# sm00thix/cvmatrix

Hardware: AMD Instinct MI355X
Metric: folds/sec (training_XTX_XTY, center+scale) at N=1e5,K=512 (higher is better)
Workload: dtype f64

## Files before the change

cvmatrix_amd/_lib.py:

```python

from __future__ import annotations

import ctypes as C
import os

import torch

_HERE = os.path.dirname(os.path.abspath(__file__))
LIB_PATH = os.environ.get("CVM_LIB_PATH") or os.path.join(_HERE, "libcvmhip.so")

CVM_OK, CVM_EINVAL, CVM_EWORKSPACE, CVM_ELAUNCH = 0, 1, 2, 3
CVM_F32, CVM_F64 = 0, 1
RET_XTX, RET_XTY = 0x01, 0x02
CENTER_X, CENTER_Y, SCALE_X, SCALE_Y = 0x04, 0x08, 0x10, 0x20
IDX_HOST = 0x40

EXPORTS = (
    "cvm_version", "cvm_source_hash", "cvm_last_error", "cvm_gstats_len", "cvm_fit_workspace_bytes",
    "cvm_gram_fit", "cvm_fold_workspace_bytes", "cvm_fold_update", "cvm_fold_update_ex", "cvm_plan_fold", "cvm_debug_force_splits", "cvm_debug_resident",
    "cvm_timing_enable", "cvm_timing_read", "cvm_timing_read_kinds", "cvm_fill_probe", "cvm_clock_probe",
    "cvm_sweep_workspace_bytes", "cvm_sweep_fit", "cvm_sweep_folds", "cvm_sweep_fold_range", "cvm_sweep_all",
    "cvm_partition_workspace_bytes", "cvm_partition_labels", "cvm_partition_periodic", "cvm_weights_check",
    "cvm_pls_workspace_bytes", "cvm_pls_fit", "cvm_pls_plan",
    "cvm_pls_sse_workspace_bytes", "cvm_pls_validation_sse",
    "cvm_ridge_workspace_bytes", "cvm_ridge_fit",
    "cvm_pcr_workspace_bytes", "cvm_pcr_fit",
    "cvm_cv_predict", "cvm_cv_predict_plan",
)

_lib = None


def load():
    global _lib
    if _lib is not None:
        return _lib
    if not os.path.exists(LIB_PATH):
        raise ImportError(
            f"{LIB_PATH} is missing: build the HIP extension first "
            "(python -m cvmatrix_amd.build, or __graft_entry__.build()). "
            "cvmatrix_amd has no CPU fallback."
        )
# ... 82 lines not shown
    lib.cvm_timing_enable.argtypes = [C.c_int]
    lib.cvm_timing_read.restype = C.c_int
    lib.cvm_timing_read.argtypes = [vp, vp, vp, vp]
    lib.cvm_timing_read_kinds.restype = C.c_int
    lib.cvm_timing_read_kinds.argtypes = [C.POINTER(C.c_double), C.POINTER(C.c_int64)]
    lib.cvm_fill_probe.restype = C.c_int
    lib.cvm_fill_probe.argtypes = [vp, sz, vp]
    lib.cvm_clock_probe.restype = C.c_int
    lib.cvm_clock_probe.argtypes = [vp, sz]
    lib.cvm_debug_force_splits.restype = C.c_int
    lib.cvm_debug_force_splits.argtypes = [C.c_int, C.c_int]
    lib.cvm_debug_resident.restype = C.c_int
    lib.cvm_debug_resident.argtypes = [C.c_int]
    lib.cvm_plan_fold.restype = C.c_int
    lib.cvm_plan_fold.argtypes = [i64, i64, C.c_int, C.c_int, C.c_int, u32, sz, vp]
    _lib = lib
    return lib


def check(rc: int, what: str) -> None:
    if rc != CVM_OK:
        msg = load().cvm_last_error().decode()
        raise RuntimeError(f"{what} failed (code {rc}): {msg}")


def ptr(t) -> int:
    if t is None:
        return 0
    if hasattr(t, "data_ptr"):
        return t.data_ptr()
# ... 2 lines not shown
```

cvmatrix_amd/csrc/cvmhip.hip:

```cpp

#include <hip/hip_runtime.h>
#include <stdint.h>
#include <stdio.h>
#include <stdlib.h>
#include <string.h>
#include <algorithm>
#include <atomic>
#include <functional>
#include <map>
#include <mutex>
#include <queue>
#include <tuple>
#include <type_traits>
#include <vector>

#include "../../include/cvmhip.h"

namespace {

#include "geometry.hpp"
#include "wgram_fallback.hpp"
#include "wgram4.hpp"
#include "finalize.hpp"
#include "colstats.hpp"
// ... 479 lines not shown
  info[3] = p.g.nT;
  info[4] = p.folds_per_batch;
  int64_t per4 = 0;
  const int es_ = dtype == CVM_F64 ? 8 : 4;
  const bool tri = ((size_t)K * es_) % 16 == 0 && (es_ == 4 || M % 2 == 0) &&
                   !(es_ == 8 && fold_mode && p.splits == 1);
  if (!p.g.diag_only) per4 += (int64_t)(p.g.nTiles - p.g.P) * 64 + (int64_t)p.g.P * (tri ? 36 : 48);
  if (M > 0) {
    if (tri && !p.g.diag_only) per4 += (int64_t)p.g.P * (M > 16 ? 16 : 8) + (int64_t)p.g.P * (p.g.Yc - 1) * 16;
    else per4 += (int64_t)p.g.P * p.g.Yc * 16;
  }
  info[5] = per4;
  return CVM_OK;
}

}
```

cvmatrix_amd/csrc/geometry.hpp:

```cpp
#pragma once

constexpr int TILE = 128;
constexpr int STAGE_ROWS = 16;
constexpr int FOLD_STAGES = 64;
constexpr int PITCH = 144;
constexpr int YT = 32;
constexpr int YPITCH = 48;
constexpr int NTHREADS = 512;
constexpr size_t LDS_BUDGET = 150 * 1024;
constexpr int PANEL_ELEMS = STAGE_ROWS * PITCH;
constexpr int BUF_ELEMS = 2 * PANEL_ELEMS + STAGE_ROWS;
constexpr int TARGET_WG_1 = 256;
constexpr int TARGET_WG_2 = 256;
constexpr int QUEUE_STRIDE = 32;
constexpr size_t QUEUE_BYTES = 8 * QUEUE_STRIDE * sizeof(unsigned);
constexpr int QUEUE_DONE = 8;

template <typename T> struct MF;
template <> struct MF<double> {
  typedef double acc_t __attribute__((ext_vector_type(4)));
  static __device__ __forceinline__ acc_t mfma(double a, double b, acc_t c) {
    return __builtin_amdgcn_mfma_f64_16x16x4f64(a, b, c, 0, 0, 0);
  }
  static __device__ __forceinline__ int drow(int lane, int r) { return (lane >> 4) + 4 * r; }
// ... 48 lines not shown
  int64_t seg0;
  int n_seg, splits;
  int s_off, s_diag;
  Geom g;
  long n_items0, ipx0;
  long n_items1, ipx1;
  unsigned *queue;
  char *ws;
  const double *fstats;
  const void *G, *H;
  void *out_XTX, *out_XTY;
  unsigned flags;
  int *stat_flags;
  int diag_first;
  int fpx;
  int *fused_status;
  unsigned long long *retry_items;
  int retry_mode;
  int test_mode;
  int32_t *status_out;
  const double *gstats;
  double ddof, resolution;
  void *out_muX, *out_sdX, *out_muY, *out_sdY;
  double *out_fold;
  int dbg;
  unsigned long long *clock_stamps;
  int clock_wgs;
};

template <typename T> __device__ __forceinline__ T *unit_tiles(char *ws, const Geom &g, long u) {
// ... 30 lines not shown
  WgramArgs<T> a;
  a.X = r->X; a.Y = r->Y; a.w = r->w; a.idx = r->idx; a.offs = r->offs;
  a.N = r->N; a.seg0 = r->seg0; a.n_seg = r->n_seg; a.splits = r->splits;
  a.s_off = r->s_off; a.s_diag = r->s_diag;
  a.g.K = r->g.K; a.g.M = r->g.M; a.g.P = r->g.P; a.g.Kp = r->g.Kp;
  a.g.Yc = r->g.Yc; a.g.Mp = r->g.Mp; a.g.nTiles = r->g.nTiles; a.g.nT = r->g.nT;
  a.g.diag_only = r->g.diag_only;
  a.g.tile_elems = r->g.tile_elems; a.g.h_elems = r->g.h_elems;
  a.g.stat_len = r->g.stat_len; a.g.unit_bytes = r->g.unit_bytes;
  a.n_items0 = r->n_items0; a.ipx0 = r->ipx0; a.n_items1 = r->n_items1; a.ipx1 = r->ipx1;
  a.queue = r->queue;
  a.ws = r->ws; a.dbg = r->dbg;
  a.fstats = r->fstats; a.G = r->G; a.H = r->H;
  a.out_XTX = r->out_XTX; a.out_XTY = r->out_XTY; a.flags = r->flags;
  a.stat_flags = r->stat_flags; a.diag_first = r->diag_first; a.gstats = r->gstats;
  a.fpx = r->fpx; a.fused_status = r->fused_status; a.retry_items = r->retry_items;
  a.retry_mode = r->retry_mode; a.test_mode = r->test_mode; a.status_out = r->status_out;
  a.ddof = r->ddof; a.resolution = r->resolution;
  a.out_muX = r->out_muX; a.out_sdX = r->out_sdX; a.out_muY = r->out_muY; a.out_sdY = r->out_sdY;
  a.out_fold = r->out_fold;
  return a;
}

__device__ __forceinline__ void decode_tile(int t, int P, int &ti, int &tj) {
  int i = 0, rem = t;
  while (rem >= P - i) { rem -= P - i; ++i; }
  ti = i; tj = i + rem;
}
__host__ __device__ __forceinline__ int tile_id(int i, int j, int P) {
  return i * P - i * (i - 1) / 2 + (j - i);
}

__device__ __forceinline__ void decode_off_tile(int k, int P, int &ti, int &tj) {
  int i = 0, rem = k;
  while (rem >= P - 1 - i) { rem -= P - 1 - i; ++i; }
  ti = i; tj = i + 1 + rem;
}

struct Item { int seg, sp, nsp, it, ti, tj, yc; long u; };
template <typename T> __device__ __forceinline__ bool decode_slot(const WgramArgs<T> &a, int xcd, long q, Item &o) {
  const Geom &g = a.g;
  long item, cu;
  int k;
  if (a.diag_first == 2) {
    const int per = g.nT;
    const long fl = q / per;
    k = (int)(q - fl * per);
    const long sg = (long)xcd * a.fpx + fl;
    if (fl >= a.fpx || sg >= a.n_seg) return false;
    const int n1 = g.P * g.Yc;
    if (k < n1) {
      if (g.diag_only) { o.ti = o.tj = k / g.Yc; o.yc = k - o.ti * g.Yc; }
      else if (k < g.P) { o.ti = o.tj = k; o.yc = 0; }
      else { const int e = k - g.P; o.ti = o.tj = e / (g.Yc - 1); o.yc = 1 + e - o.ti * (g.Yc - 1); }
      o.it = tile_id(o.ti, o.ti, g.P);
    } else {
      decode_off_tile(k - n1, g.P, o.ti, o.tj);
      o.yc = 0;
      o.it = tile_id(o.ti, o.tj, g.P);
    }
    o.seg = uni((int)sg); o.sp = 0; o.nsp = 1; o.it = uni(o.it);
    o.ti = uni(o.ti); o.tj = uni(o.tj); o.yc = uni(o.yc);
    o.u = (long)o.seg * a.splits;
    return true;
  }
  if (a.diag_first) q = q < a.ipx1 ? q + a.ipx0 : q - a.ipx1;
  if (q < a.ipx0) {
    item = (long)xcd * a.ipx0 + q;
    if (item >= a.n_items0) return false;
    const int per = g.nTiles - g.P;
    cu = item / per; k = (int)(item - cu * per);
    o.nsp = a.s_off;
    decode_off_tile(k, g.P, o.ti, o.tj);
    o.yc = 0;
    o.it = tile_id(o.ti, o.tj, g.P);
  } else {
    const long q1 = q - a.ipx0;
    if (q1 >= a.ipx1) return false;
    item = (long)xcd * a.ipx1 + q1;
    if (item >= a.n_items1) return false;
    const int per = g.P * g.Yc;
    cu = item / per; k = (int)(item - cu * per);
    o.nsp = a.s_diag;
    if (g.diag_only) { o.ti = o.tj = k / g.Yc; o.yc = k - o.ti * g.Yc; }
    else if (k < g.P) { o.ti = o.tj = k; o.yc = 0; }
    else { const int e = k - g.P; o.ti = o.tj = e / (g.Yc - 1); o.yc = 1 + e - o.ti * (g.Yc - 1); }
    o.it = tile_id(o.ti, o.ti, g.P);
  }
  o.seg = (int)(cu / o.nsp);
  o.sp = (int)(cu - (long)o.seg * o.nsp);
  o.seg = uni(o.seg); o.sp = uni(o.sp); o.nsp = uni(o.nsp); o.it = uni(o.it);
  o.ti = uni(o.ti); o.tj = uni(o.tj); o.yc = uni(o.yc);
  o.u = (long)o.seg * a.splits + o.sp;
  return true;
}
template <typename T> __device__ __forceinline__ bool decode_item(const WgramArgs<T> &a, long b, Item &o) {
  const long b0 = 8 * a.ipx0;
  if (b < b0) return decode_slot(a, (int)(b & 7), b >> 3, o);
  const long bb = b - b0;
  return decode_slot(a, (int)(bb & 7), a.ipx0 + (bb >> 3), o);
}

__device__ __forceinline__ void split_range(int64_t n, int splits, int sp, int64_t &r0, int64_t &r1) {
  int64_t per = (n + splits - 1) / splits;
  per = (per + STAGE_ROWS - 1) / STAGE_ROWS * STAGE_ROWS;
  r0 = (int64_t)sp * per; if (r0 > n) r0 = n;
  r1 = r0 + per; if (r1 > n) r1 = n;
}

__device__ __forceinline__ void wait_vmcnt_le(int n) {
#define CVM_W(k) case k: asm volatile("s_waitcnt vmcnt(" #k ")" ::: "memory"); break;
  switch (n) {
    CVM_W(0) CVM_W(1) CVM_W(2) CVM_W(3) CVM_W(4) CVM_W(5) CVM_W(6) CVM_W(7) CVM_W(8)
    CVM_W(9) CVM_W(10) CVM_W(11) CVM_W(12) CVM_W(13) CVM_W(14) CVM_W(15)
    default: asm volatile("s_waitcnt vmcnt(16)" ::: "memory"); break;
  }
#undef CVM_W
}

__device__ __forceinline__ void dma16_lanes(const void *src, unsigned lds_addr) {
  unsigned keep;
  asm volatile("s_mov_b32 %0, m0\n\ts_mov_b32 m0, %2\n\ts_nop 0\n\t"
// ... 4 lines not shown
```

cvmatrix_amd/csrc/host.hpp:

```cpp
#pragma once

thread_local char g_err[512] = "";
int fail(int code, const char *fmt, const char *detail = "") {
  snprintf(g_err, sizeof(g_err), fmt, detail);
  return code;
}
#define HIP_OK(expr)                                                             \
  do {                                                                           \
    hipError_t e_ = (expr);                                                      \
    if (e_ != hipSuccess) return fail(CVM_ELAUNCH, #expr ": %s", hipGetErrorString(e_)); \
  } while (0)

struct TimedLaunch { hipEvent_t a, b; int kind; };
constexpr int MAX_TIMED = 8192;
std::atomic<bool> g_timing{false};
std::mutex g_timing_mu;
TimedLaunch g_timed[MAX_TIMED];
int g_ntimed = 0;
inline TimedLaunch *timed_begin(int kind, hipStream_t st) {
  if (!g_timing.load(std::memory_order_relaxed)) return nullptr;
  TimedLaunch *tl = nullptr;
  {
    std::lock_guard<std::mutex> lk(g_timing_mu);
    if (g_ntimed >= MAX_TIMED) return nullptr;
// ... 194 lines not shown
  const int esize = dtype == CVM_F64 ? 8 : 4;
  const int diag_only = fold_mode && !(flags & CVM_RET_XTX);
  p.g = make_geom(K, M, esize, diag_only);
  const SplitChoice c = choose_splits2(n_folds, max_rows, p.g, esize, target_wg(K, M, esize));
  set_plan_splits(p, c.s_off, c.s_diag);
  p.fstat_bytes_per_fold = fold_mode ? align_up(fstat_len(K, M) * 8, 256) : 0;
  for (;;) {
    const size_t per_fold = (size_t)p.splits * p.g.unit_bytes + p.fstat_bytes_per_fold;
    int64_t nb = (int64_t)(ws_bytes / per_fold);
    if (nb >= 1) { p.folds_per_batch = nb < n_folds ? nb : n_folds; return CVM_OK; }
    if (p.splits == 1) return CVM_EWORKSPACE;
    set_plan_splits(p, (p.s_off + 1) / 2, (p.s_diag + 1) / 2);
  }
}

template <typename T> void set_items(WgramArgs<T> &a, const Plan &p, int64_t n_seg) {
  const Geom &g = p.g;
  a.n_seg = (int)n_seg; a.splits = p.splits; a.s_off = p.s_off; a.s_diag = p.s_diag; a.g = g;
  const int per0 = g.diag_only ? 0 : g.nTiles - g.P, per1 = g.P * g.Yc;
  a.n_items0 = (long)n_seg * p.s_off * per0;
  a.n_items1 = (long)n_seg * p.s_diag * per1;
  a.ipx0 = (a.n_items0 + 7) / 8;
  a.ipx1 = (a.n_items1 + 7) / 8;
}
void set_fin_splits(FinArgs &f, const Plan &p, int n_sum) {
  f.splits = p.splits; f.s_off = p.s_off; f.s_diag = p.s_diag; f.n_sum = n_sum;
}

template <typename T> bool wgram4_ok(const WgramArgs<T> &a, bool aligned) {
  static const bool force_fallback = getenv("CVM_FORCE_FALLBACK") && atoi(getenv("CVM_FORCE_FALLBACK")) != 0;
  if (force_fallback || !aligned) return false;
  if (sizeof(T) == 8)
    return (a.g.M % 2 == 0) && ((uintptr_t)a.Y % 16 == 0) && ((uintptr_t)a.w % 8 == 0);
  return ((uintptr_t)a.Y % 4 == 0) && ((uintptr_t)a.w % 4 == 0);
}

struct WsCarve { size_t usable; unsigned *queue; };
WsCarve carve_queue(void *ws, size_t ws_bytes) {
// ... 543 lines not shown
template <typename T>
WgramArgs<T> fused_args(const FoldCall &c, const Plan &p, int64_t f0, int64_t nb, const double *fstats) {
  WgramArgs<T> a;
  memset(&a, 0, sizeof(a));
  a.X = (const T *)c.X; a.Y = (const T *)c.Y; a.w = (const T *)c.w;
  a.idx = c.idx; a.offs = c.offsets; a.N = c.N; a.seg0 = f0;
  set_items(a, p, nb);
  a.ws = nullptr;
  a.fstats = fstats; a.G = c.G; a.H = c.H;
  a.out_XTX = c.out_XTX; a.out_XTY = c.want_xty ? c.out_XTY : nullptr; a.flags = c.flags;
  if (fold_switches().fused_order == 2) {
    a.diag_first = 2;
    a.fpx = (int)((nb + 7) / 8);
    const int per0 = p.g.diag_only ? 0 : p.g.nTiles - p.g.P, per1 = p.g.P * p.g.Yc;
    a.ipx0 = (long)a.fpx * per0; a.ipx1 = (long)a.fpx * per1;
  }
  return a;
}

template <typename T>
int fold_update_impl(const void *X, const void *Y, const void *w, const int64_t *idx,
                     const int64_t *offsets, const int64_t *host_offsets, int64_t n_folds, int64_t N,
                     int K, int M, int dtype, unsigned flags, double ddof, double resolution,
                     const void *G, const void *H, const double *gstats, void *out_XTX,
                     void *out_XTY, void *out_muX, void *out_sdX, void *out_muY, void *out_sdY,
                     double *out_fold, void *ws, size_t ws_bytes, hipStream_t st, int32_t *status) {
  int64_t max_rows = 0;
  for (int64_t f = 0; f < n_folds; ++f) {
    const int64_t n = host_offsets[f + 1] - host_offsets[f];
    if (n < 0) return fail(CVM_EINVAL, "cvm_fold_update: offsets must be non-decreasing%s");
// ... 269 lines not shown
```

cvmatrix_amd/csrc/wgram4.hpp:

```cpp
#pragma once

constexpr int NT4 = 512;
template <typename T> __device__ __forceinline__ void partial_store(T *p, T v) { *p = v; }
constexpr int NBUF4 = 4;
constexpr size_t LDS4_BYTES = (size_t)NBUF4 * BUF_ELEMS * 8;
template <typename T> constexpr size_t lds4_bytes() { return (size_t)NBUF4 * BUF_ELEMS * sizeof(T); }

__host__ __device__ inline size_t fstat_len(int K, int M);
template <typename T> struct FusedPre;
template <typename T>
__device__ __forceinline__ void fused_g_preload32(FusedPre<T> &p, int a0, int b0, int K, const T *Gt, int lane, int row_lo);
template <typename T, int TP>
__device__ __forceinline__ void fused_finish_direct32(T (*Ts)[TP], const double *rs, int a0, int b0, int K, T *out,
                                                      double swt, bool cX, bool sX, int lane, int row_lo,
                                                      const FusedPre<T> &p);
template <typename T, int TP>
__device__ __forceinline__ void fused_finish_block(T (*Ts)[TP], const double *rs, bool diagb, int a0,
                                                   int b0, int K, const T *Gt, T *out,
                                                   double swt, bool cX, bool sX, int lane);
template <typename T, int TP>
__device__ __forceinline__ void fused_finish_direct(T (*Ts)[TP], const double *rs, bool diagb, int a0,
                                                    int b0, int K, const T *Gt, T *out,
                                                    double swt, bool cX, bool sX, int lane, int row_lo, int row_hi);
template <typename T, int TP>
// ... 56 lines not shown
      mark = FUSED_SKIP;
    } else {
      if (fused_status) __hip_atomic_fetch_add(fused_status + 1, 1, __ATOMIC_RELAXED, __HIP_MEMORY_SCOPE_AGENT);
      mark = FUSED_POISON;
    }
    asm volatile("s_waitcnt vmcnt(0)" ::: "memory");
  }
  *reinterpret_cast<volatile int *>(smem_raw + fused_launch_lds_bytes<T>() - 16) = mark;
}
template <typename T> __device__ __forceinline__ int fused_mark(const int *stat_flags, const char *smem_raw) {
  if (!stat_flags) return FUSED_GO;
  return uni(*reinterpret_cast<const volatile int *>(smem_raw + fused_launch_lds_bytes<T>() - 16));
}

template <typename T, bool WEIGHTED, bool GATHER, bool HWR, bool MFMR, int ROLER, bool FUSEDR = false>
__device__ __noinline__ ROLE_ATTR void wgram4_body(kargs_ptr<T> kargs, int xcd_q, int slot_q) {
  typedef typename MF<T>::acc_t acc_t;
#ifdef CVM_STAMPS
  const unsigned long long c_entry = __builtin_amdgcn_s_memtime();
#endif
  const WgramArgs<T> a = kernel_args<T>(kargs);
  extern __shared__ __attribute__((aligned(16))) char smem_raw[];
  T *smem = reinterpret_cast<T *>(smem_raw);
  const Geom &g = a.g;
  const int tid = threadIdx.x;
  const int lane = tid & 63;
  const int wave_all = __builtin_amdgcn_readfirstlane(tid >> 6);
  const int wave = wave_all & 3;

  Item wi;
  if (!decode_slot(a, uni(xcd_q), (long)uni(slot_q), wi)) ROLE_EXIT();
  const long u = wi.u;
  const int it = wi.it, seg = wi.seg, sp = wi.sp, ti = wi.ti, tj = wi.tj, yc = wi.yc;
  const bool diag = (ti == tj);
  const int wr = wave >> 1, wc = wave & 1;
  const bool h_wave = diag && wave == 2;
  const bool do_g = !g.diag_only && yc == 0;

  int64_t seg_begin, seg_rows;
  if (a.offs) { seg_begin = a.offs[a.seg0 + seg]; seg_rows = a.offs[a.seg0 + seg + 1] - seg_begin; }
  else { seg_begin = 0; seg_rows = a.N; }
  int64_t r0, r1;
  split_range(seg_rows, wi.nsp, sp, r0, r1);
  r0 = uni64(r0); r1 = uni64(r1); seg_begin = uni64(seg_begin);
  const int nstages = uni((int)((r1 - r0 + STAGE_ROWS - 1) / STAGE_ROWS));
  const int colA0 = uni(ti * TILE), colB0 = uni(tj * TILE);

  if (ROLER == 3) {
    const int d = wave_all - 4;
    const char *zero_src = reinterpret_cast<const char *>(unip(g_zero_line));
    constexpr unsigned ES = sizeof(T);
    constexpr int EPL = 16 / (int)ES;
    const char *one_src = reinterpret_cast<const char *>(ES == 8 ? (const void *)unip(g_one_line)
                                                                : (const void *)unip(g_one_line_f));
    int oa = EPL * lane, ob = EPL * lane, oy = ES == 8 ? 2 * (lane & 15) : (lane & 31);
    if (colA0 + oa > g.K - EPL) oa = g.K - EPL - colA0;
    if (colB0 + ob > g.K - EPL) ob = g.K - EPL - colB0;
    if (oa < 0) oa = 0;
    if (ob < 0) ob = 0;
    const int ycol0 = yc * YT;
// ... 601 lines not shown
  int n = 0;
  for (int q = 0; q < t.na; ++q) t.rd[n++] = t.at[q];
  for (int j = 0; j < t.nf; ++j) {
    bool is_a = false;
    for (int q = 0; q < t.na; ++q) is_a = is_a || t.at[q] == j;
    if (!is_a) t.rd[n++] = j;
  }
  return t;
}
constexpr bool diag_ystat_wave(int W, int NBY) {
  const DiagTab t = diag_tab(W, NBY == 1);
  return t.ws || t.ys[0] || (NBY > 1 && t.ys[1]);
}

template <typename T, bool WEIGHTED, bool GATHER, int W, int NBY, bool YSTAT, bool FUSEDR = false>
__device__ __noinline__ ROLE_ATTR void wgram4_diag_body(kargs_ptr<T> kargs, int xcd_q, int slot_q) {
  typedef typename MF<T>::acc_t acc_t;
#ifdef CVM_STAMPS
  const unsigned long long c_entry = __builtin_amdgcn_s_memtime();
#endif
  const WgramArgs<T> a = kernel_args<T>(kargs);
  extern __shared__ __attribute__((aligned(16))) char smem_raw[];
  T *smem = reinterpret_cast<T *>(smem_raw);
  const Geom &g = a.g;
  const int lane = threadIdx.x & 63;
  Item wi;
  decode_slot(a, uni(xcd_q), (long)uni(slot_q), wi);
  const long u = wi.u;
  const int it = wi.it, seg = wi.seg, sp = wi.sp, ti = wi.ti;
  int64_t seg_begin, seg_rows;
  if (a.offs) { seg_begin = a.offs[a.seg0 + seg]; seg_rows = a.offs[a.seg0 + seg + 1] - seg_begin; }
  else { seg_begin = 0; seg_rows = a.N; }
  int64_t r0, r1;
  split_range(seg_rows, wi.nsp, sp, r0, r1);
  r0 = uni64(r0); r1 = uni64(r1);
  const int nstages = uni((int)((r1 - r0 + STAGE_ROWS - 1) / STAGE_ROWS));

  constexpr DiagTab P = diag_tab(W, NBY == 1);
  constexpr int NF = P.nf, NA = P.na, NG = P.ng, NX = P.nx;
  acc_t acc[NG], acch[NX * NBY];
#pragma unroll
  for (int i = 0; i < NG; ++i) acc[i] = (acc_t){0, 0, 0, 0};
#pragma unroll
  for (int i = 0; i < NX * NBY; ++i) acch[i] = (acc_t){0, 0, 0, 0};
  constexpr bool TWO_LEVEL = sizeof(T) == 4;
  acc_t acc2[TWO_LEVEL ? NG : 1], acch2[TWO_LEVEL ? NX * NBY : 1];
  if (TWO_LEVEL) {
#pragma unroll
    for (int i = 0; i < NG; ++i) acc2[i] = (acc_t){0, 0, 0, 0};
#pragma unroll
    for (int i = 0; i < NX * NBY; ++i) acch2[i] = (acc_t){0, 0, 0, 0};
// ... 319 lines not shown
    asm volatile("s_waitcnt vmcnt(0)" ::: "memory");
    const unsigned long long c_exit = __builtin_amdgcn_s_memtime();
    if (lane == 0 && uni(slot_q) < CVM_ITEM_STAMP_STRIDE) {
      unsigned long long *o = g_stamps5 + ((size_t)(uni(xcd_q) * CVM_ITEM_STAMP_STRIDE + uni(slot_q)) * 4 + W) * 8;
      o[0] = c_entry; o[1] = c_loop0 - c_entry; o[2] = c_loop1 - c_loop0; o[3] = t_b; o[4] = t_c;
      o[5] = (unsigned long long)nstages;
      o[6] = (unsigned long long)(ti | (ti << 8)) | ((unsigned long long)blockIdx.x << 32);
      o[7] = c_exit;
    }
  }
#endif
  ROLE_EXIT();
}

template <typename T, bool WEIGHTED, bool GATHER, bool FUSED>
__device__ __forceinline__ void wgram4_item(const WgramArgs<T> &a, kargs_ptr<T> kargs, const Item &wi, int wave_all,
                                            int xq, int sq) {
  const Geom &g = a.g;
  const int wave = wave_all & 3;
  if (wave_all >= 4) { wgram4_body<T, WEIGHTED, GATHER, false, false, 3, FUSED>(kargs, xq, sq); return; }
  const int ti = wi.ti, tj = wi.tj, yc = wi.yc;
  const bool diag = (ti == tj);
  const bool do_g = !g.diag_only && yc == 0;
  if (FUSED && diag && do_g) {
    const bool wide = g.M > 16;
    const bool ys = a.stat_flags != nullptr;
#define CVM_DIAGF(WV)                                                                                            \
    do {                                                                                                         \
      if (wide) {                                                                                                \
        if (ys) wgram4_diag_body<T, WEIGHTED, GATHER, WV, 2, diag_ystat_wave(WV, 2), true>(kargs, xq, sq);       \
        else wgram4_diag_body<T, WEIGHTED, GATHER, WV, 2, false, true>(kargs, xq, sq);                           \
      } else {                                                                                                   \
        if (ys) wgram4_diag_body<T, WEIGHTED, GATHER, WV, 1, diag_ystat_wave(WV, 1), true>(kargs, xq, sq);       \
        else wgram4_diag_body<T, WEIGHTED, GATHER, WV, 1, false, true>(kargs, xq, sq);                           \
      }                                                                                                          \
    } while (0)
    if (wave == 0) CVM_DIAGF(0);
    else if (wave == 1) CVM_DIAGF(1);
    else if (wave == 2) CVM_DIAGF(2);
    else CVM_DIAGF(3);
#undef CVM_DIAGF
    return;
  }
  if (FUSED) {
    if (diag && wave == 2) wgram4_body<T, WEIGHTED, GATHER, true, true, 0, true>(kargs, xq, sq);
    else if (do_g) wgram4_body<T, WEIGHTED, GATHER, false, true, 0, true>(kargs, xq, sq);
    else wgram4_body<T, WEIGHTED, GATHER, false, false, 0, true>(kargs, xq, sq);
    return;
  }
  if (diag && do_g) {
    const bool wide = g.M > 16, ys = (ti == 0);
#define CVM_DIAG(WV)                                                                                             \
    do {                                                                                                         \
      if (wide) {                                                                                                \
        if (ys) wgram4_diag_body<T, WEIGHTED, GATHER, WV, 2, diag_ystat_wave(WV, 2)>(kargs, xq, sq);             \
        else wgram4_diag_body<T, WEIGHTED, GATHER, WV, 2, false>(kargs, xq, sq);                                 \
      } else {                                                                                                   \
        if (ys) wgram4_diag_body<T, WEIGHTED, GATHER, WV, 1, diag_ystat_wave(WV, 1)>(kargs, xq, sq);             \
        else wgram4_diag_body<T, WEIGHTED, GATHER, WV, 1, false>(kargs, xq, sq);                                 \
      }                                                                                                          \
    } while (0)
    if (wave == 0) CVM_DIAG(0);
    else if (wave == 1) CVM_DIAG(1);
    else if (wave == 2) CVM_DIAG(2);
    else CVM_DIAG(3);
#undef CVM_DIAG
    return;
  }
  const int role = !diag ? 0 : ((yc == 0 && (wave == 0 || wave == 3)) ? 1 : ((ti == 0 && wave == 1) ? 2 : 0));
  if (diag && wave == 2) wgram4_body<T, WEIGHTED, GATHER, true, true, 0>(kargs, xq, sq);
  else if (role == 1) { if (do_g) wgram4_body<T, WEIGHTED, GATHER, false, true, 1>(kargs, xq, sq); else wgram4_body<T, WEIGHTED, GATHER, false, false, 1>(kargs, xq, sq); }
  else if (role == 2) { if (do_g) wgram4_body<T, WEIGHTED, GATHER, false, true, 2>(kargs, xq, sq); else wgram4_body<T, WEIGHTED, GATHER, false, false, 2>(kargs, xq, sq); }
  else { if (do_g) wgram4_body<T, WEIGHTED, GATHER, false, true, 0>(kargs, xq, sq); else wgram4_body<T, WEIGHTED, GATHER, false, false, 0>(kargs, xq, sq); }
}

__device__ __forceinline__ int fetch_position(unsigned *queue, int xcd) {
  return (int)__hip_atomic_fetch_add(queue + xcd * QUEUE_STRIDE, 1u, __ATOMIC_RELAXED, __HIP_MEMORY_SCOPE_AGENT);
}
template <typename T, bool WEIGHTED, bool GATHER, bool FUSED = false>
__global__ __launch_bounds__(NT4, 2) void wgram4_kernel(const WgramArgs<T> a) {
  __shared__ int s_next[2][2];
  const kargs_ptr<T> kargs = kernarg_address<T>();
  const int wave_all = __builtin_amdgcn_readfirstlane(threadIdx.x >> 6);
  unsigned xcc;
  asm volatile("s_getreg_b32 %0, hwreg(HW_REG_XCC_ID)" : "=s"(xcc));
  const int home = (int)(xcc & 7u);
  const long per_xcd = a.ipx0 + a.ipx1;
  auto fetch = [&](int &fx, int &fq, int &probe) {
    Item tmp;
    if (FUSED && a.retry_mode) {
      const int q = fetch_position(a.queue, 0);
      const int n = __hip_atomic_load(a.fused_status, __ATOMIC_RELAXED, __HIP_MEMORY_SCOPE_AGENT);
      if (q < n) {
        const unsigned long long it = __hip_atomic_load(a.retry_items + q, __ATOMIC_RELAXED, __HIP_MEMORY_SCOPE_AGENT);
        fx = (int)(it >> 32); fq = (int)(it & 0xffffffffu);
      } else { fx = -1; fq = 0; }
      return;
    }
    while (probe < 8) {
      const int x = (home + probe) & 7;
      const int q = fetch_position(a.queue, x);
      if (q >= per_xcd) { ++probe; continue; }
      if (decode_slot(a, x, (long)q, tmp)) { fx = x; fq = q; return; }
    }
    fx = -1; fq = 0;
  };
  const bool clk = a.clock_stamps && threadIdx.x == 0 && (int)blockIdx.x < a.clock_wgs;
  if (clk) {
    const unsigned long long c0 = __builtin_amdgcn_s_memtime(), q0 = __builtin_amdgcn_s_memrealtime();
    a.clock_stamps[4 * blockIdx.x + 0] = c0; a.clock_stamps[4 * blockIdx.x + 1] = q0;
  }
  int probe = 0;
  if (threadIdx.x == 4 * 64) {
    int fx, fq;
    fetch(fx, fq, probe);
    s_next[0][0] = fx; s_next[0][1] = fq;
  }
  __syncthreads();
#ifdef CVM_STAMPS
  const unsigned long long c0 = __builtin_amdgcn_s_memtime(), q0 = __builtin_amdgcn_s_memrealtime();
#endif
  for (int n = 0;; ++n) {
    const int xq = uni(s_next[n & 1][0]), sq = uni(s_next[n & 1][1]);
    if (xq < 0) break;
    Item wi;
    decode_slot(a, xq, (long)sq, wi);
    wgram4_item<T, WEIGHTED, GATHER, FUSED>(a, kargs, wi, wave_all, xq, sq);
    if (threadIdx.x == 4 * 64) {
      int fx, fq;
      fetch(fx, fq, probe);
      s_next[(n + 1) & 1][0] = fx; s_next[(n + 1) & 1][1] = fq;
    }
    lds_barrier();
  }
  if (clk) {
    const unsigned long long c1 = __builtin_amdgcn_s_memtime(), q1 = __builtin_amdgcn_s_memrealtime();
    a.clock_stamps[4 * blockIdx.x + 2] = c1; a.clock_stamps[4 * blockIdx.x + 3] = q1;
  }
  if (threadIdx.x == 0) {
    const unsigned left = __hip_atomic_fetch_add(a.queue + QUEUE_DONE, 1u, __ATOMIC_RELAXED, __HIP_MEMORY_SCOPE_AGENT);
    if (left == gridDim.x - 1) {
#pragma unroll
      for (int x = 0; x < 8; ++x)
        __hip_atomic_store(a.queue + x * QUEUE_STRIDE, 0u, __ATOMIC_RELAXED, __HIP_MEMORY_SCOPE_AGENT);
      __hip_atomic_store(a.queue + QUEUE_DONE, 0u, __ATOMIC_RELAXED, __HIP_MEMORY_SCOPE_AGENT);
      if (FUSED && a.retry_mode && a.status_out) {
// ... 23 lines not shown
```

include/cvmhip.h:

```cpp
#ifndef CVMHIP_H
#define CVMHIP_H

#include <stddef.h>
#include <stdint.h>

#ifdef __cplusplus
extern "C" {
#endif

#define CVM_OK 0
#define CVM_EINVAL 1
#define CVM_EWORKSPACE 2
#define CVM_ELAUNCH 3

#define CVM_F32 0
#define CVM_F64 1

#define CVM_RET_XTX 0x01u
#define CVM_RET_XTY 0x02u
#define CVM_CENTER_X 0x04u
#define CVM_CENTER_Y 0x08u
#define CVM_SCALE_X 0x10u
#define CVM_SCALE_Y 0x20u
#define CVM_IDX_HOST 0x40u
// ... 90 lines not shown
int cvm_timing_enable(int on);
int cvm_timing_read(double *ms_fit, int64_t *n_fit, double *ms_fold, int64_t *n_fold);
int cvm_timing_read_kinds(double *ms4, int64_t *n4);

int cvm_fill_probe(void *buf, size_t bytes, void *stream);

int cvm_clock_probe(void *device_buf, size_t bytes);

int cvm_debug_force_splits(int s_off, int s_diag);

int cvm_debug_resident(int mode);

int cvm_plan_fold(int64_t n_folds, int64_t max_fold_rows, int K, int M, int dtype,
                  unsigned flags, size_t ws_bytes, int64_t *info);

#ifdef __cplusplus
}
#endif
#endif
```

Baseline: 21280.

## Decode work items once in fetcher thread and broadcast full descriptor via LDS

The fetching thread now fully decodes each work item (tile, segment, split, row range, stage count) into an 80-byte descriptor stored in shared memory. Every wave then reads it with vector LDS loads instead of redoing the integer division and offset lookups. Divisions use 32-bit unsigned arithmetic when a new 'narrow' flag shows the sizes fit. The intent is to cut scalar decode and global offset-load latency per item, at the cost of more LDS traffic and a larger serial step in the fetcher thread. A host-side describe API is added for testing.

After: 21350 (median of 6 runs). No clear change (+0.3%).

```diff
diff --git a/cvmatrix_amd/_lib.py b/cvmatrix_amd/_lib.py
--- a/cvmatrix_amd/_lib.py
+++ b/cvmatrix_amd/_lib.py
@@ -25,7 +25,7 @@
     "cvm_pls_sse_workspace_bytes", "cvm_pls_validation_sse",
     "cvm_ridge_workspace_bytes", "cvm_ridge_fit",
     "cvm_pcr_workspace_bytes", "cvm_pcr_fit",
-    "cvm_cv_predict", "cvm_cv_predict_plan",
+    "cvm_cv_predict", "cvm_cv_predict_plan", "cvm_describe_items",
 )
 
 _lib = None
@@ -138,6 +138,9 @@
     lib.cvm_debug_resident.argtypes = [C.c_int]
     lib.cvm_plan_fold.restype = C.c_int
     lib.cvm_plan_fold.argtypes = [i64, i64, C.c_int, C.c_int, C.c_int, u32, sz, vp]
+    lib.cvm_describe_items.restype = C.c_int
+    lib.cvm_describe_items.argtypes = [i64, vp, i64, i64, C.c_int, C.c_int, C.c_int, C.c_int, C.c_int, C.c_int,
+                                       C.c_int, i64, i64, vp, vp]
     _lib = lib
     return lib
 
diff --git a/cvmatrix_amd/csrc/cvmhip.hip b/cvmatrix_amd/csrc/cvmhip.hip
--- a/cvmatrix_amd/csrc/cvmhip.hip
+++ b/cvmatrix_amd/csrc/cvmhip.hip
@@ -517,4 +517,40 @@
   return CVM_OK;
 }
 
-}
+int cvm_describe_items(int64_t n_seg, const int64_t *host_offsets, int64_t N, int64_t seg0, int K, int M,
+                       int diag_only, int s_off, int s_diag, int diag_first, int wide, int64_t q0, int64_t nq,
+                       int64_t *out, int64_t *info) {
+  if (!info || (nq > 0 && !out) || K <= 0 || M < 0 || n_seg < 1 || n_seg > 0x7fffffff || s_off < 1 || s_diag < 1 ||
+      s_off > 65535 || s_diag > 65535 || diag_first < 0 || diag_first > 2 || q0 < 0 || nq < 0 || seg0 < 0 ||
+      (diag_first == 2 && (s_off != 1 || s_diag != 1)) || (!host_offsets && n_seg != 1))
+    return fail(CVM_EINVAL, "cvm_describe_items: bad argument%s");
+  Plan p;
+  p.g = make_geom(K, M, 8, diag_only);
+  set_plan_splits(p, s_off, s_diag);
+  WgramArgs<double> a;
+  memset(&a, 0, sizeof(a));
+  a.N = N; a.seg0 = seg0;
+  set_items(a, p, n_seg);
+  a.diag_first = diag_first;
+  if (diag_first == 2) {
+    a.fpx = (int)((n_seg + 7) / 8);
+    const int per0 = p.g.diag_only ? 0 : p.g.nTiles - p.g.P, per1 = p.g.P * p.g.Yc;
+    a.ipx0 = (long)a.fpx * per0; a.ipx1 = (long)a.fpx * per1;
+    set_narrow(a);
+  }
+  if (wide) a.narrow = 0;
+  info[0] = a.ipx0 + a.ipx1; info[1] = a.n_items0; info[2] = a.ipx0; info[3] = a.n_items1; info[4] = a.ipx1;
+  info[5] = a.narrow; info[6] = a.fpx; info[7] = a.splits;
+  for (int x = 0; x < 8; ++x)
+    for (int64_t i = 0; i < nq; ++i) {
+      ItemDesc d;
+      describe_item(a, host_offsets, x, (long)(q0 + i), d);
+      int64_t *o = out + ((size_t)x * nq + i) * 16;
+      o[0] = d.valid; o[1] = d.xcd; o[2] = d.q; o[3] = d.seg; o[4] = d.sp; o[5] = d.nsp; o[6] = d.it; o[7] = d.ti;
+      o[8] = d.tj; o[9] = d.yc; o[10] = d.nstages; o[11] = d.pad_; o[12] = d.u; o[13] = d.seg_begin; o[14] = d.r0;
+      o[15] = d.r1;
+    }
+  return CVM_OK;
+}
+
+}
diff --git a/cvmatrix_amd/csrc/geometry.hpp b/cvmatrix_amd/csrc/geometry.hpp
--- a/cvmatrix_amd/csrc/geometry.hpp
+++ b/cvmatrix_amd/csrc/geometry.hpp
@@ -86,6 +86,7 @@
   int *stat_flags;
   int diag_first;
   int fpx;
+  int narrow;
   int *fused_status;
   unsigned long long *retry_items;
   int retry_mode;
@@ -146,7 +147,7 @@
   a.fstats = r->fstats; a.G = r->G; a.H = r->H;
   a.out_XTX = r->out_XTX; a.out_XTY = r->out_XTY; a.flags = r->flags;
   a.stat_flags = r->stat_flags; a.diag_first = r->diag_first; a.gstats = r->gstats;
-  a.fpx = r->fpx; a.fused_status = r->fused_status; a.retry_items = r->retry_items;
+  a.fpx = r->fpx; a.narrow = r->narrow; a.fused_status = r->fused_status; a.retry_items = r->retry_items;
   a.retry_mode = r->retry_mode; a.test_mode = r->test_mode; a.status_out = r->status_out;
   a.ddof = r->ddof; a.resolution = r->resolution;
   a.out_muX = r->out_muX; a.out_sdX = r->out_sdX; a.out_muY = r->out_muY; a.out_sdY = r->out_sdY;
@@ -163,20 +164,26 @@
   return i * P - i * (i - 1) / 2 + (j - i);
 }
 
-__device__ __forceinline__ void decode_off_tile(int k, int P, int &ti, int &tj) {
+__host__ __device__ __forceinline__ void decode_off_tile(int k, int P, int &ti, int &tj) {
   int i = 0, rem = k;
   while (rem >= P - 1 - i) { rem -= P - 1 - i; ++i; }
   ti = i; tj = i + 1 + rem;
 }
 
+__host__ __device__ __forceinline__ long div_nn(long a, long b, bool narrow) {
+  return narrow ? (long)((unsigned)a / (unsigned)b) : a / b;
+}
+
 struct Item { int seg, sp, nsp, it, ti, tj, yc; long u; };
-template <typename T> __device__ __forceinline__ bool decode_slot(const WgramArgs<T> &a, int xcd, long q, Item &o) {
+template <typename T>
+__host__ __device__ __forceinline__ bool decode_position(const WgramArgs<T> &a, int xcd, long q, Item &o) {
   const Geom &g = a.g;
+  const bool narrow = a.narrow != 0;
   long item, cu;
   int k;
   if (a.diag_first == 2) {
     const int per = g.nT;
-    const long fl = q / per;
+    const long fl = div_nn(q, per, narrow);
     k = (int)(q - fl * per);
     const long sg = (long)xcd * a.fpx + fl;
     if (fl >= a.fpx || sg >= a.n_seg) return false;
@@ -191,17 +198,19 @@
       o.yc = 0;
       o.it = tile_id(o.ti, o.tj, g.P);
     }
-    o.seg = uni((int)sg); o.sp = 0; o.nsp = 1; o.it = uni(o.it);
-    o.ti = uni(o.ti); o.tj = uni(o.tj); o.yc = uni(o.yc);
+    o.seg = (int)sg; o.sp = 0; o.nsp = 1;
     o.u = (long)o.seg * a.splits;
     return true;
   }
-  if (a.diag_first) q = q < a.ipx1 ? q + a.ipx0 : q - a.ipx1;
+  if (a.diag_first) {
+    if (q >= a.ipx0 + a.ipx1) return false;
+    q = q < a.ipx1 ? q + a.ipx0 : q - a.ipx1;
+  }
   if (q < a.ipx0) {
     item = (long)xcd * a.ipx0 + q;
     if (item >= a.n_items0) return false;
     const int per = g.nTiles - g.P;
-    cu = item / per; k = (int)(item - cu * per);
+    cu = div_nn(item, per, narrow); k = (int)(item - cu * per);
     o.nsp = a.s_off;
     decode_off_tile(k, g.P, o.ti, o.tj);
     o.yc = 0;
@@ -212,32 +221,85 @@
     item = (long)xcd * a.ipx1 + q1;
     if (item >= a.n_items1) return false;
     const int per = g.P * g.Yc;
-    cu = item / per; k = (int)(item - cu * per);
+    cu = div_nn(item, per, narrow); k = (int)(item - cu * per);
     o.nsp = a.s_diag;
     if (g.diag_only) { o.ti = o.tj = k / g.Yc; o.yc = k - o.ti * g.Yc; }
     else if (k < g.P) { o.ti = o.tj = k; o.yc = 0; }
     else { const int e = k - g.P; o.ti = o.tj = e / (g.Yc - 1); o.yc = 1 + e - o.ti * (g.Yc - 1); }
     o.it = tile_id(o.ti, o.ti, g.P);
   }
-  o.seg = (int)(cu / o.nsp);
+  o.seg = (int)div_nn(cu, o.nsp, narrow);
   o.sp = (int)(cu - (long)o.seg * o.nsp);
+  o.u = (long)o.seg * a.splits + o.sp;
+  return true;
+}
+template <typename T> __device__ __forceinline__ bool decode_item(const WgramArgs<T> &a, long b, Item &o) {
+  const long b0 = 8 * a.ipx0;
+  const long bb = b - b0;
+  if (!(b < b0 ? decode_position(a, (int)(b & 7), b >> 3, o) : decode_position(a, (int)(bb & 7), a.ipx0 + (bb >> 3), o)))
+    return false;
   o.seg = uni(o.seg); o.sp = uni(o.sp); o.nsp = uni(o.nsp); o.it = uni(o.it);
   o.ti = uni(o.ti); o.tj = uni(o.tj); o.yc = uni(o.yc);
   o.u = (long)o.seg * a.splits + o.sp;
   return true;
 }
-template <typename T> __device__ __forceinline__ bool decode_item(const WgramArgs<T> &a, long b, Item &o) {
-  const long b0 = 8 * a.ipx0;
-  if (b < b0) return decode_slot(a, (int)(b & 7), b >> 3, o);
-  const long bb = b - b0;
-  return decode_slot(a, (int)(bb & 7), a.ipx0 + (bb >> 3), o);
-}
-
-__device__ __forceinline__ void split_range(int64_t n, int splits, int sp, int64_t &r0, int64_t &r1) {
-  int64_t per = (n + splits - 1) / splits;
+
+__host__ __device__ __forceinline__ void split_range(int64_t n, int splits, int sp, int64_t &r0, int64_t &r1,
+                                                     bool narrow = false) {
+  int64_t per = div_nn(n + splits - 1, splits, narrow);
   per = (per + STAGE_ROWS - 1) / STAGE_ROWS * STAGE_ROWS;
   r0 = (int64_t)sp * per; if (r0 > n) r0 = n;
   r1 = r0 + per; if (r1 > n) r1 = n;
+}
+
+struct ItemDesc {
+  int valid;
+  int xcd, q;
+  int seg, sp, nsp;
+  int it, ti, tj, yc;
+  int nstages;
+  int pad_;
+  long long u;
+  long long seg_begin;
+  long long r0, r1;
+};
+static_assert(sizeof(ItemDesc) == 80, "ItemDesc: five 16-byte pieces");
+template <typename T>
+__host__ __device__ __forceinline__ void describe_item(const WgramArgs<T> &a, const int64_t *offs, int xcd, long q,
+                                                       ItemDesc &d) {
+  Item o;
+  d.xcd = xcd; d.q = (int)q; d.pad_ = 0;
+  d.valid = decode_position(a, xcd, q, o) ? 1 : 0;
+  if (!d.valid) {
+    d.seg = d.sp = d.nsp = d.it = d.ti = d.tj = d.yc = d.nstages = 0;
+    d.u = d.seg_begin = d.r0 = d.r1 = 0;
+    return;
+  }
+  d.seg = o.seg; d.sp = o.sp; d.nsp = o.nsp; d.it = o.it; d.ti = o.ti; d.tj = o.tj; d.yc = o.yc; d.u = o.u;
+  int64_t seg_begin, seg_rows;
+  if (offs) { seg_begin = offs[a.seg0 + o.seg]; seg_rows = offs[a.seg0 + o.seg + 1] - seg_begin; }
+  else { seg_begin = 0; seg_rows = a.N; }
+  const bool narrow = a.narrow && seg_rows >= 0 && seg_rows < ((int64_t)1 << 30);
+  int64_t r0, r1;
+  split_range(seg_rows, o.nsp, o.sp, r0, r1, narrow);
+  d.seg_begin = seg_begin; d.r0 = r0; d.r1 = r1;
+  d.nstages = (int)((r1 - r0 + STAGE_ROWS - 1) / STAGE_ROWS);
+}
+typedef const __attribute__((address_space(3))) ItemDesc *desc_ptr;
+__device__ __forceinline__ ItemDesc load_desc(desc_ptr p) {
+  p = (desc_ptr)(uintptr_t)(unsigned)uni((int)(unsigned)(uintptr_t)p);
+  typedef int v4i __attribute__((ext_vector_type(4)));
+  const __attribute__((address_space(3))) v4i *v = (const __attribute__((address_space(3))) v4i *)p;
+  v4i r[sizeof(ItemDesc) / 16];
+#pragma unroll
+  for (unsigned i = 0; i < sizeof(ItemDesc) / 16; ++i) r[i] = v[i];
+  ItemDesc d;
+  __builtin_memcpy(&d, r, sizeof(d));
+  d.valid = uni(d.valid); d.xcd = uni(d.xcd); d.q = uni(d.q);
+  d.seg = uni(d.seg); d.sp = uni(d.sp); d.nsp = uni(d.nsp);
+  d.it = uni(d.it); d.ti = uni(d.ti); d.tj = uni(d.tj); d.yc = uni(d.yc); d.nstages = uni(d.nstages);
+  d.u = uni64(d.u); d.seg_begin = uni64(d.seg_begin); d.r0 = uni64(d.r0); d.r1 = uni64(d.r1);
+  return d;
 }
 
 __device__ __forceinline__ void wait_vmcnt_le(int n) {
diff --git a/cvmatrix_amd/csrc/host.hpp b/cvmatrix_amd/csrc/host.hpp
--- a/cvmatrix_amd/csrc/host.hpp
+++ b/cvmatrix_amd/csrc/host.hpp
@@ -232,6 +232,12 @@
   }
 }
 
+template <typename T> void set_narrow(WgramArgs<T> &a) {
+  const long lim = (long)1 << 31;
+  const long per_xcd = a.diag_first == 2 ? (long)a.fpx * a.g.nT : a.ipx0 + a.ipx1;
+  a.narrow = a.n_items0 < lim && a.n_items1 < lim && per_xcd < lim / 8 &&
+             (long)a.n_seg * a.splits < lim && a.s_off < (1 << 15) && a.s_diag < (1 << 15);
+}
 template <typename T> void set_items(WgramArgs<T> &a, const Plan &p, int64_t n_seg) {
   const Geom &g = p.g;
   a.n_seg = (int)n_seg; a.splits = p.splits; a.s_off = p.s_off; a.s_diag = p.s_diag; a.g = g;
@@ -240,6 +246,7 @@
   a.n_items1 = (long)n_seg * p.s_diag * per1;
   a.ipx0 = (a.n_items0 + 7) / 8;
   a.ipx1 = (a.n_items1 + 7) / 8;
+  set_narrow(a);
 }
 void set_fin_splits(FinArgs &f, const Plan &p, int n_sum) {
   f.splits = p.splits; f.s_off = p.s_off; f.s_diag = p.s_diag; f.n_sum = n_sum;
@@ -813,6 +820,7 @@
     a.fpx = (int)((nb + 7) / 8);
     const int per0 = p.g.diag_only ? 0 : p.g.nTiles - p.g.P, per1 = p.g.P * p.g.Yc;
     a.ipx0 = (long)a.fpx * per0; a.ipx1 = (long)a.fpx * per1;
+    set_narrow(a);
   }
   return a;
 }
diff --git a/cvmatrix_amd/csrc/wgram4.hpp b/cvmatrix_amd/csrc/wgram4.hpp
--- a/cvmatrix_amd/csrc/wgram4.hpp
+++ b/cvmatrix_amd/csrc/wgram4.hpp
@@ -94,7 +94,7 @@
 }
 
 template <typename T, bool WEIGHTED, bool GATHER, bool HWR, bool MFMR, int ROLER, bool FUSEDR = false>
-__device__ __noinline__ ROLE_ATTR void wgram4_body(kargs_ptr<T> kargs, int xcd_q, int slot_q) {
+__device__ __noinline__ ROLE_ATTR void wgram4_body(kargs_ptr<T> kargs, desc_ptr desc) {
   typedef typename MF<T>::acc_t acc_t;
 #ifdef CVM_STAMPS
   const unsigned long long c_entry = __builtin_amdgcn_s_memtime();
@@ -108,22 +108,19 @@
   const int wave_all = __builtin_amdgcn_readfirstlane(tid >> 6);
   const int wave = wave_all & 3;
 
-  Item wi;
-  if (!decode_slot(a, uni(xcd_q), (long)uni(slot_q), wi)) ROLE_EXIT();
+  const ItemDesc wi = load_desc(desc);
+  if (!wi.valid) ROLE_EXIT();
   const long u = wi.u;
   const int it = wi.it, seg = wi.seg, sp = wi.sp, ti = wi.ti, tj = wi.tj, yc = wi.yc;
+  const int xcd_q = wi.xcd, slot_q = wi.q;
+  (void)xcd_q; (void)slot_q;
   const bool diag = (ti == tj);
   const int wr = wave >> 1, wc = wave & 1;
   const bool h_wave = diag && wave == 2;
   const bool do_g = !g.diag_only && yc == 0;
 
-  int64_t seg_begin, seg_rows;
-  if (a.offs) { seg_begin = a.offs[a.seg0 + seg]; seg_rows = a.offs[a.seg0 + seg + 1] - seg_begin; }
-  else { seg_begin = 0; seg_rows = a.N; }
-  int64_t r0, r1;
-  split_range(seg_rows, wi.nsp, sp, r0, r1);
-  r0 = uni64(r0); r1 = uni64(r1); seg_begin = uni64(seg_begin);
-  const int nstages = uni((int)((r1 - r0 + STAGE_ROWS - 1) / STAGE_ROWS));
+  const int64_t seg_begin = wi.seg_begin, r0 = wi.r0, r1 = wi.r1;
+  const int nstages = wi.nstages;
   const int colA0 = uni(ti * TILE), colB0 = uni(tj * TILE);
 
   if (ROLER == 3) {
@@ -755,7 +752,7 @@
 }
 
 template <typename T, bool WEIGHTED, bool GATHER, int W, int NBY, bool YSTAT, bool FUSEDR = false>
-__device__ __noinline__ ROLE_ATTR void wgram4_diag_body(kargs_ptr<T> kargs, int xcd_q, int slot_q) {
+__device__ __noinline__ ROLE_ATTR void wgram4_diag_body(kargs_ptr<T> kargs, desc_ptr desc) {
   typedef typename MF<T>::acc_t acc_t;
 #ifdef CVM_STAMPS
   const unsigned long long c_entry = __builtin_amdgcn_s_memtime();
@@ -765,17 +762,13 @@
   T *smem = reinterpret_cast<T *>(smem_raw);
   const Geom &g = a.g;
   const int lane = threadIdx.x & 63;
-  Item wi;
-  decode_slot(a, uni(xcd_q), (long)uni(slot_q), wi);
+  const ItemDesc wi = load_desc(desc);
   const long u = wi.u;
   const int it = wi.it, seg = wi.seg, sp = wi.sp, ti = wi.ti;
-  int64_t seg_begin, seg_rows;
-  if (a.offs) { seg_begin = a.offs[a.seg0 + seg]; seg_rows = a.offs[a.seg0 + seg + 1] - seg_begin; }
-  else { seg_begin = 0; seg_rows = a.N; }
-  int64_t r0, r1;
-  split_range(seg_rows, wi.nsp, sp, r0, r1);
-  r0 = uni64(r0); r1 = uni64(r1);
-  const int nstages = uni((int)((r1 - r0 + STAGE_ROWS - 1) / STAGE_ROWS));
+  const int xcd_q = wi.xcd, slot_q = wi.q;
+  (void)xcd_q; (void)slot_q;
+  const int64_t seg_begin = wi.seg_begin, r0 = wi.r0, r1 = wi.r1;
+  const int nstages = wi.nstages;
 
   constexpr DiagTab P = diag_tab(W, NBY == 1);
   constexpr int NF = P.nf, NA = P.na, NG = P.ng, NX = P.nx;
@@ -1125,11 +1118,11 @@
 }
 
 template <typename T, bool WEIGHTED, bool GATHER, bool FUSED>
-__device__ __forceinline__ void wgram4_item(const WgramArgs<T> &a, kargs_ptr<T> kargs, const Item &wi, int wave_all,
-                                            int xq, int sq) {
+__device__ __forceinline__ void wgram4_item(const WgramArgs<T> &a, kargs_ptr<T> kargs, const ItemDesc &wi, int wave_all,
+                                            desc_ptr desc) {
   const Geom &g = a.g;
   const int wave = wave_all & 3;
-  if (wave_all >= 4) { wgram4_body<T, WEIGHTED, GATHER, false, false, 3, FUSED>(kargs, xq, sq); return; }
+  if (wave_all >= 4) { wgram4_body<T, WEIGHTED, GATHER, false, false, 3, FUSED>(kargs, desc); return; }
   const int ti = wi.ti, tj = wi.tj, yc = wi.yc;
   const bool diag = (ti == tj);
   const bool do_g = !g.diag_only && yc == 0;
@@ -1139,11 +1132,11 @@
 #define CVM_DIAGF(WV)                                                                                            \
     do {                                                                                                         \
       if (wide) {                                                                                                \
-        if (ys) wgram4_diag_body<T, WEIGHTED, GATHER, WV, 2, diag_ystat_wave(WV, 2), true>(kargs, xq, sq);       \
-        else wgram4_diag_body<T, WEIGHTED, GATHER, WV, 2, false, true>(kargs, xq, sq);                           \
+        if (ys) wgram4_diag_body<T, WEIGHTED, GATHER, WV, 2, diag_ystat_wave(WV, 2), true>(kargs, desc);         \
+        else wgram4_diag_body<T, WEIGHTED, GATHER, WV, 2, false, true>(kargs, desc);                             \
       } else {                                                                                                   \
-        if (ys) wgram4_diag_body<T, WEIGHTED, GATHER, WV, 1, diag_ystat_wave(WV, 1), true>(kargs, xq, sq);       \
-        else wgram4_diag_body<T, WEIGHTED, GATHER, WV, 1, false, true>(kargs, xq, sq);                           \
+        if (ys) wgram4_diag_body<T, WEIGHTED, GATHER, WV, 1, diag_ystat_wave(WV, 1), true>(kargs, desc);         \
+        else wgram4_diag_body<T, WEIGHTED, GATHER, WV, 1, false, true>(kargs, desc);                             \
       }                                                                                                          \
     } while (0)
     if (wave == 0) CVM_DIAGF(0);
@@ -1154,9 +1147,9 @@
     return;
   }
   if (FUSED) {
-    if (diag && wave == 2) wgram4_body<T, WEIGHTED, GATHER, true, true, 0, true>(kargs, xq, sq);
-    else if (do_g) wgram4_body<T, WEIGHTED, GATHER, false, true, 0, true>(kargs, xq, sq);
-    else wgram4_body<T, WEIGHTED, GATHER, false, false, 0, true>(kargs, xq, sq);
+    if (diag && wave == 2) wgram4_body<T, WEIGHTED, GATHER, true, true, 0, true>(kargs, desc);
+    else if (do_g) wgram4_body<T, WEIGHTED, GATHER, false, true, 0, true>(kargs, desc);
+    else wgram4_body<T, WEIGHTED, GATHER, false, false, 0, true>(kargs, desc);
     return;
   }
   if (diag && do_g) {
@@ -1164,11 +1157,11 @@
 #define CVM_DIAG(WV)                                                                                             \
     do {                                                                                                         \
       if (wide) {                                                                                                \
-        if (ys) wgram4_diag_body<T, WEIGHTED, GATHER, WV, 2, diag_ystat_wave(WV, 2)>(kargs, xq, sq);             \
-        else wgram4_diag_body<T, WEIGHTED, GATHER, WV, 2, false>(kargs, xq, sq);                                 \
+        if (ys) wgram4_diag_body<T, WEIGHTED, GATHER, WV, 2, diag_ystat_wave(WV, 2)>(kargs, desc);               \
+        else wgram4_diag_body<T, WEIGHTED, GATHER, WV, 2, false>(kargs, desc);                                   \
       } else {                                                                                                   \
-        if (ys) wgram4_diag_body<T, WEIGHTED, GATHER, WV, 1, diag_ystat_wave(WV, 1)>(kargs, xq, sq);             \
-        else wgram4_diag_body<T, WEIGHTED, GATHER, WV, 1, false>(kargs, xq, sq);                                 \
+        if (ys) wgram4_diag_body<T, WEIGHTED, GATHER, WV, 1, diag_ystat_wave(WV, 1)>(kargs, desc);               \
+        else wgram4_diag_body<T, WEIGHTED, GATHER, WV, 1, false>(kargs, desc);                                   \
       }                                                                                                          \
     } while (0)
     if (wave == 0) CVM_DIAG(0);
@@ -1179,10 +1172,10 @@
     return;
   }
   const int role = !diag ? 0 : ((yc == 0 && (wave == 0 || wave == 3)) ? 1 : ((ti == 0 && wave == 1) ? 2 : 0));
-  if (diag && wave == 2) wgram4_body<T, WEIGHTED, GATHER, true, true, 0>(kargs, xq, sq);
-  else if (role == 1) { if (do_g) wgram4_body<T, WEIGHTED, GATHER, false, true, 1>(kargs, xq, sq); else wgram4_body<T, WEIGHTED, GATHER, false, false, 1>(kargs, xq, sq); }
-  else if (role == 2) { if (do_g) wgram4_body<T, WEIGHTED, GATHER, false, true, 2>(kargs, xq, sq); else wgram4_body<T, WEIGHTED, GATHER, false, false, 2>(kargs, xq, sq); }
-  else { if (do_g) wgram4_body<T, WEIGHTED, GATHER, false, true, 0>(kargs, xq, sq); else wgram4_body<T, WEIGHTED, GATHER, false, false, 0>(kargs, xq, sq); }
+  if (diag && wave == 2) wgram4_body<T, WEIGHTED, GATHER, true, true, 0>(kargs, desc);
+  else if (role == 1) { if (do_g) wgram4_body<T, WEIGHTED, GATHER, false, true, 1>(kargs, desc); else wgram4_body<T, WEIGHTED, GATHER, false, false, 1>(kargs, desc); }
+  else if (role == 2) { if (do_g) wgram4_body<T, WEIGHTED, GATHER, false, true, 2>(kargs, desc); else wgram4_body<T, WEIGHTED, GATHER, false, false, 2>(kargs, desc); }
+  else { if (do_g) wgram4_body<T, WEIGHTED, GATHER, false, true, 0>(kargs, desc); else wgram4_body<T, WEIGHTED, GATHER, false, false, 0>(kargs, desc); }
 }
 
 __device__ __forceinline__ int fetch_position(unsigned *queue, int xcd) {
@@ -1190,31 +1183,33 @@
 }
 template <typename T, bool WEIGHTED, bool GATHER, bool FUSED = false>
 __global__ __launch_bounds__(NT4, 2) void wgram4_kernel(const WgramArgs<T> a) {
-  __shared__ int s_next[2][2];
+  __shared__ __attribute__((aligned(16))) ItemDesc s_desc[2];
   const kargs_ptr<T> kargs = kernarg_address<T>();
   const int wave_all = __builtin_amdgcn_readfirstlane(threadIdx.x >> 6);
   unsigned xcc;
   asm volatile("s_getreg_b32 %0, hwreg(HW_REG_XCC_ID)" : "=s"(xcc));
   const int home = (int)(xcc & 7u);
   const long per_xcd = a.ipx0 + a.ipx1;
-  auto fetch = [&](int &fx, int &fq, int &probe) {
-    Item tmp;
+  auto fetch = [&](ItemDesc &d, int &probe) {
     if (FUSED && a.retry_mode) {
       const int q = fetch_position(a.queue, 0);
       const int n = __hip_atomic_load(a.fused_status, __ATOMIC_RELAXED, __HIP_MEMORY_SCOPE_AGENT);
       if (q < n) {
         const unsigned long long it = __hip_atomic_load(a.retry_items + q, __ATOMIC_RELAXED, __HIP_MEMORY_SCOPE_AGENT);
-        fx = (int)(it >> 32); fq = (int)(it & 0xffffffffu);
-      } else { fx = -1; fq = 0; }
+        describe_item(a, a.offs, (int)(it >> 32), (long)(int)(it & 0xffffffffu), d);
+        if (d.valid) return;
+      }
+      d = ItemDesc{}; d.xcd = -1;
       return;
     }
     while (probe < 8) {
       const int x = (home + probe) & 7;
       const int q = fetch_position(a.queue, x);
       if (q >= per_xcd) { ++probe; continue; }
-      if (decode_slot(a, x, (long)q, tmp)) { fx = x; fq = q; return; }
-    }
-    fx = -1; fq = 0;
+      describe_item(a, a.offs, x, (long)q, d);
+      if (d.valid) return;
+    }
+    d = ItemDesc{}; d.xcd = -1;
   };
   const bool clk = a.clock_stamps && threadIdx.x == 0 && (int)blockIdx.x < a.clock_wgs;
   if (clk) {
@@ -1223,24 +1218,23 @@
   }
   int probe = 0;
   if (threadIdx.x == 4 * 64) {
-    int fx, fq;
-    fetch(fx, fq, probe);
-    s_next[0][0] = fx; s_next[0][1] = fq;
+    ItemDesc d;
+    fetch(d, probe);
+    s_desc[0] = d;
   }
   __syncthreads();
 #ifdef CVM_STAMPS
   const unsigned long long c0 = __builtin_amdgcn_s_memtime(), q0 = __builtin_amdgcn_s_memrealtime();
 #endif
   for (int n = 0;; ++n) {
-    const int xq = uni(s_next[n & 1][0]), sq = uni(s_next[n & 1][1]);
-    if (xq < 0) break;
-    Item wi;
-    decode_slot(a, xq, (long)sq, wi);
-    wgram4_item<T, WEIGHTED, GATHER, FUSED>(a, kargs, wi, wave_all, xq, sq);
+    const desc_ptr desc = (desc_ptr)&s_desc[n & 1];
+    const ItemDesc wi = load_desc(desc);
+    if (wi.xcd < 0) break;
+    wgram4_item<T, WEIGHTED, GATHER, FUSED>(a, kargs, wi, wave_all, desc);
     if (threadIdx.x == 4 * 64) {
-      int fx, fq;
-      fetch(fx, fq, probe);
-      s_next[(n + 1) & 1][0] = fx; s_next[(n + 1) & 1][1] = fq;
+      ItemDesc d;
+      fetch(d, probe);
+      s_desc[(n + 1) & 1] = d;
     }
     lds_barrier();
   }
diff --git a/include/cvmhip.h b/include/cvmhip.h
--- a/include/cvmhip.h
+++ b/include/cvmhip.h
@@ -128,6 +128,10 @@
 int cvm_plan_fold(int64_t n_folds, int64_t max_fold_rows, int K, int M, int dtype,
                   unsigned flags, size_t ws_bytes, int64_t *info);
 
+int cvm_describe_items(int64_t n_seg, const int64_t *host_offsets, int64_t N, int64_t seg0, int K, int M,
+                       int diag_only, int s_off, int s_diag, int diag_first, int wide, int64_t q0, int64_t nq,
+                       int64_t *out, int64_t *info);
+
 #ifdef __cplusplus
 }
 #endif
```
